# nsdumont/Semantic-Spiking-Neural-SLAM-2023

Measured on AMD Instinct MI355X. Metric: sim-sec/wall-sec, SSP-SLAM ssp_dim=1015 10k PI neurons, 1/2/4/8 MI355X, higher is better.
Workload: dtype f32; 1 GPU; PathIntegration 2-D ssp_dim=1015 pi_n_neurons=10000/VCO (508 VCOs, 5080000 LIF neurons), configs[1]; eval_points_per_vco=4000, parallelism=1 GPU, build_cache=miss

## Files before the change

semantic-spiking-neural-slam-2023_amd/csrc/ssn_block.hpp:

```cpp
#pragma once
#include <type_traits>
#include "ssn_launch.hpp"

namespace ssn {

__device__ inline float wave_sum_dpp(float v) {
  int x;
#define SSN_DPP_ADD(ctrl, rmask)                                                                             \
  x = __builtin_amdgcn_update_dpp(0, __builtin_bit_cast(int, v), ctrl, rmask, 0xF, false);                    \
  v += __builtin_bit_cast(float, x);
  SSN_DPP_ADD(0xB1, 0xF)
  SSN_DPP_ADD(0x4E, 0xF)
  SSN_DPP_ADD(0x141, 0xF)
  SSN_DPP_ADD(0x140, 0xF)
  SSN_DPP_ADD(0x142, 0xA)
  SSN_DPP_ADD(0x143, 0xC)
#undef SSN_DPP_ADD
  return v;
}
__device__ inline float row_sum_dpp(float v) {
  int x;
#define SSN_DPP_ADD(ctrl)                                                                                    \
  x = __builtin_amdgcn_update_dpp(0, __builtin_bit_cast(int, v), ctrl, 0xF, 0xF, false);                      \
  v += __builtin_bit_cast(float, x);
// ... 10 lines not shown
  }
  SSN_DPP_STAGE(0xB1, 0xF) SSN_DPP_STAGE(0x4E, 0xF) SSN_DPP_STAGE(0x141, 0xF) SSN_DPP_STAGE(0x140, 0xF)
  SSN_DPP_STAGE(0x142, 0xA) SSN_DPP_STAGE(0x143, 0xC)
#undef SSN_DPP_STAGE
}
__device__ inline double wave_sum_dpp(double v) {
#pragma unroll
  for (int off = 32; off > 0; off >>= 1) v += __shfl_xor(v, off, 64);
  return v;
}
template <int N>
__device__ inline void wave_sum_dpp_n(double* v) {
#pragma unroll
  for (int r = 0; r < N; ++r) v[r] = wave_sum_dpp(v[r]);
}

typedef float f32x2 __attribute__((ext_vector_type(2)));
typedef unsigned int u32x2 __attribute__((ext_vector_type(2)));
__device__ inline f32x2 pk_clamp01(f32x2 x) {
  f32x2 r;
  asm("v_pk_mul_f32 %0, %1, 1.0 op_sel_hi:[1,0] clamp" : "=v"(r) : "v"(x));
  return r;
}
__device__ inline f32x2 pk_sub_clamp01(f32x2 x, f32x2 y) {
  f32x2 r;
  asm("v_pk_add_f32 %0, %1, %2 neg_lo:[0,1] neg_hi:[0,1] clamp" : "=v"(r) : "v"(x), "s"(y));
  return r;
}
__device__ inline f32x2 pk_mul_clamp01(f32x2 x, f32x2 y) {
  f32x2 r;
  asm("v_pk_mul_f32 %0, %1, %2 clamp" : "=v"(r) : "v"(x), "s"(y));
  return r;
}
__device__ inline f32x2 pk_fma_clamp01_vsv(f32x2 x, f32x2 y, f32x2 z) {
  f32x2 r;
  asm("v_pk_fma_f32 %0, %1, %2, %3 clamp" : "=v"(r) : "v"(x), "s"(y), "v"(z));
  return r;
}
__device__ inline f32x2 pk_fma_clamp01_trans_vvs(f32x2 x, f32x2 y, f32x2 z) {
  f32x2 r;
  asm("s_nop 0\n\tv_pk_fma_f32 %0, %1, %2, %3 clamp" : "=v"(r) : "v"(x), "v"(y), "s"(z));
  return r;
}

__device__ inline f32x2 pk_fma_clamp01_vs_negv(f32x2 x, f32x2 y, f32x2 z) {
  f32x2 r;
  asm("v_pk_fma_f32 %0, %1, %2, %3 neg_lo:[0,0,1] neg_hi:[0,0,1] clamp" : "=v"(r) : "v"(x), "s"(y), "v"(z));
  return r;
}

struct LifConstV3 { float na, ca, m1, c1, c2, c3, p0, p1, p2, ktau_ref, K; };
struct LifConstV3P { f32x2 na, ca, m1, c1, c2, c3, p0, p1, p2, ktau_ref; };

__device__ inline LifConstV3 lif_const_v3(double dt, double tau_rc, double tau_ref) {
  double K = 1.0;
  while (2.0 * K * tau_ref <= 1.0 && K < 1048576.0) K *= 2.0;
  while (K * tau_ref > 1.0) K *= 0.5;
  const double h = dt / tau_rc;
  const double x0 = h, x1 = 0.5 * h, x2 = 0.0669872981077807 * h;
  auto f = [](double x) { return -expm1(-x) / x; };
  const double f0 = f(x0), f1 = f(x1), f2 = f(x2);
  const double d01 = (f1 - f0) / (x1 - x0), d12 = (f2 - f1) / (x2 - x1), d012 = (d12 - d01) / (x2 - x0);
  const double q2 = d012, q1 = d01 - d012 * (x0 + x1), q0 = f0 - d01 * x0 + d012 * x0 * x1;
  LifConstV3 c;
  const float a = (float)(1.0 / (K * dt));
  float ca = a + 1.0f;
  if ((double)ca < (double)a + 1.0) ca = __builtin_bit_cast(float, __builtin_bit_cast(unsigned int, ca) + 1u);
  c.na = -a; c.ca = ca; c.m1 = (float)(1.0 + K * dt);
  c.c1 = (float)(q0 * h); c.c2 = (float)(q1 * h * h); c.c3 = (float)(q2 * h * h * h);
  {
    const double um = -expm1(-h);
    const double u0 = um * 0.9330127018922193, u1 = um * 0.5, u2 = um * 0.0669872981077807;
    auto phi = [](double u) { return log1p(-u) / u; };
    const double g0 = phi(u0), g1 = phi(u1), g2 = phi(u2);
    const double e01 = (g1 - g0) / (u1 - u0), e12 = (g2 - g1) / (u2 - u1), e012 = (e12 - e01) / (u2 - u0);
    const double r2 = e012, r1 = e01 - e012 * (u0 + u1), r0 = g0 - e01 * u0 + e012 * u0 * u1;
    c.p0 = (float)(K * tau_rc * r0); c.p1 = (float)(K * tau_rc * r1); c.p2 = (float)(K * tau_rc * r2);
  }
  c.ktau_ref = (float)(K * tau_ref); c.K = (float)K;
  return c;
}

__device__ inline f32x2 lif_state_dl(f32x2 w, f32x2 na, f32x2 ca) {
  return pk_fma_clamp01_vsv(w, (f32x2)(na), (f32x2)(ca));
}
__device__ inline f32x2 lif_state_p1(f32x2 dl, f32x2 c3, f32x2 c2) {
  f32x2 P;
  asm("v_pk_fma_f32 %0, %1, %2, %3" : "=v"(P) : "v"(dl), "v"((f32x2)(c3)), "s"((f32x2)(c2)));
  return P;
}
__device__ inline f32x2 lif_state_p2(f32x2 dl, f32x2 P, f32x2 c1) {
  asm("v_pk_fma_f32 %0, %1, %2, %3" : "=v"(P) : "v"(dl), "v"(P), "s"((f32x2)(c1)));
  return P;
}
__device__ inline void lif_state_part(f32x2 w, const LifConstV3P& c, f32x2& W0, f32x2& em) {
  W0 = pk_clamp01(w);
  const f32x2 dl = lif_state_dl(w, c.na, c.ca);
  const f32x2 P = lif_state_p2(dl, lif_state_p1(dl, c.c3, c.c2), c.c1);
  em = dl * P;
}
__device__ inline f32x2 lif_spike_test(f32x2 Jm1, f32x2 w, f32x2 W0, f32x2 em, const LifConstV3P& c, f32x2 big, f32x2& U, f32x2& nmt) {
  nmt = pk_sub_clamp01(w, (f32x2)(c.m1));
  U = __builtin_elementwise_fma(Jm1 + W0, em, -W0);
  return pk_mul_clamp01(U, big);
}
__device__ inline void lif_finish_spiking(f32x2 Jm1, f32x2& w, f32x2 U, f32x2 nmt, f32x2 spk, const LifConstV3P& c, f32x2 big) {
  f32x2 rc;
  rc.x = __builtin_amdgcn_rcpf(Jm1.x);
  rc.y = __builtin_amdgcn_rcpf(Jm1.y);
  const f32x2 u = U * rc;
  f32x2 P, nu;
  asm("v_pk_fma_f32 %0, %1, %2, %3" : "=v"(P) : "v"(u), "v"((f32x2)(c.p2)), "s"((f32x2)(c.p1)));
  asm("v_pk_fma_f32 %0, %1, %2, %3" : "=v"(P) : "v"(u), "v"(P), "s"((f32x2)(c.p0)));
  asm("v_pk_fma_f32 %0, %1, %2, %3 clamp" : "=v"(nu) : "v"(u), "v"(P), "s"((f32x2)(c.ktau_ref)));
  const f32x2 Wn = pk_fma_clamp01_vs_negv(spk, big, U);
  w = __builtin_elementwise_fma(spk, nu, Wn + nmt);
}
__device__ inline void lif_finish_silent(f32x2& w, f32x2 U, f32x2 nmt) {
  f32x2 Wn;
  asm("v_pk_mul_f32 %0, %1, -1.0 op_sel_hi:[1,0] clamp" : "=v"(Wn) : "v"(U));
  w = Wn + nmt;
}
__device__ inline f32x2 lif_input_part(f32x2 Jm1, f32x2& w, f32x2 W0, f32x2 em, const LifConstV3P& c, f32x2 big) {
  const f32x2 nmt = pk_sub_clamp01(w, (f32x2)(c.m1));
  const f32x2 U = __builtin_elementwise_fma(Jm1 + W0, em, -W0);
  const f32x2 spk = pk_mul_clamp01(U, big);
  f32x2 rc;
  rc.x = __builtin_amdgcn_rcpf(Jm1.x);
  rc.y = __builtin_amdgcn_rcpf(Jm1.y);
  f32x2 Wn, u, P, nu;
  asm("v_pk_fma_f32 %0, %2, %3, %4 neg_lo:[0,0,1] neg_hi:[0,0,1] clamp\n\t"
      "v_pk_mul_f32 %1, %4, %5"
      : "=&v"(Wn), "=v"(u)
      : "v"(spk), "s"(big), "v"(U), "v"(rc));
  asm("v_pk_fma_f32 %0, %1, %2, %3" : "=v"(P) : "v"(u), "v"((f32x2)(c.p2)), "s"((f32x2)(c.p1)));
  asm("v_pk_fma_f32 %0, %1, %2, %3" : "=v"(P) : "v"(u), "v"(P), "s"((f32x2)(c.p0)));
  asm("v_pk_fma_f32 %0, %1, %2, %3 clamp" : "=v"(nu) : "v"(u), "v"(P), "s"((f32x2)(c.ktau_ref)));
  w = __builtin_elementwise_fma(spk, nu, Wn + nmt);
  return spk;
}
__device__ inline float lif_word_in(float s, float K) { return __builtin_fmaf(-s, s < 0.0f ? K : 1.0f, 1.0f); }
__device__ inline float lif_word_out(float w, float K) { return (1.0f - w) * (w > 1.0f ? 1.0f / K : 1.0f); }

__device__ inline float bits_f(unsigned int x) { return __builtin_bit_cast(float, x); }
__device__ inline unsigned int f_bits(float x) { return __builtin_bit_cast(unsigned int, x); }

#ifdef SSN_BLOCK_STAMPS
__device__ unsigned long long g_block_stamps[9];
inline hipError_t read_block_stamps(unsigned long long* out, int reset) {
  hipError_t e = hipMemcpyFromSymbol(out, HIP_SYMBOL(g_block_stamps), sizeof(unsigned long long) * 9);
  if (e == hipSuccess && reset) {
    const unsigned long long z[9] = {0, 0, 0, 0, 0, 0, 0, 0, 0};
    e = hipMemcpyToSymbol(HIP_SYMBOL(g_block_stamps), z, sizeof z);
  }
  return e;
}
#define SSN_BSTAMP(var)                                                                          \
  do {                                                                                           \
    __builtin_amdgcn_sched_barrier(0);                                                           \
    asm volatile("s_memtime %0\n\ts_waitcnt lgkmcnt(0)" : "=s"(var) :: "memory");                \
    __builtin_amdgcn_sched_barrier(0);                                                           \
  } while (0)
#define SSN_BSTAMP_ADD(i, a, b) bst[i] += (b) - (a)
#else
#define SSN_BSTAMP(var) do {} while (0)
#define SSN_BSTAMP_ADD(i, a, b) do {} while (0)
#endif

#ifndef SSN_BLOCK_SKIP
#define SSN_BLOCK_SKIP 0
#endif
#ifndef SSN_BLOCK_PIPE
#define SSN_BLOCK_PIPE 1
#endif
#ifndef SSN_BLOCK_HOIST_A
#define SSN_BLOCK_HOIST_A 2
#endif
#ifndef SSN_BLOCK_HOIST_B
#define SSN_BLOCK_HOIST_B 4
#endif
#ifndef SSN_BLOCK_HOIST_C
#define SSN_BLOCK_HOIST_C 2
#endif
struct BlockHoist { int a, b, c; };
constexpr BlockHoist block_hoist(bool pipe, int tpb, int ng) {
  if (!pipe || SSN_BLOCK_SKIP != 0) return {0, 0, 0};
  const int room = tpb <= 512 && ng >= 10 ? ng : 0;
  const int c = SSN_BLOCK_HOIST_C >= 2 && room >= 2 ? 2 : 0;
  int b = SSN_BLOCK_HOIST_B < room - c ? SSN_BLOCK_HOIST_B : room - c;
  int a_ = SSN_BLOCK_HOIST_A < room - c - b ? SSN_BLOCK_HOIST_A : room - c - b;
  return {a_, b, c};
}

template <typename T, int DIN, int DOUT, int NPT, int TPB, int LDSW, int SPLIT = 0, int TAP = 0>
__global__ __launch_bounds__(TPB) void k_ens_block(BlockArgs<T> a) {
  static_assert(!(SPLIT && TAP), "the split kernel has no tapped form");
  constexpr bool ENC_LDS = LDSW == DIN;
  static_assert(LDSW == 0 || LDSW == DIN, "LDSW");
  extern __shared__ __align__(16) unsigned char ssn_block_dyn[];
  T* const e_lds = reinterpret_cast<T*>(ssn_block_dyn);
  constexpr bool F32 = sizeof(T) == 4;
  constexpr int PK = F32 ? 2 : 1;
  constexpr int NG = NPT / PK;
  static_assert(NPT % PK == 0, "f32 variants handle neuron pairs");
  constexpr bool PIPE = F32 && NG >= 5 && SSN_BLOCK_PIPE != 0;
  constexpr BlockHoist HO = block_hoist(PIPE, TPB, NG);
  constexpr int HC = HO.c, HA = HO.a, HB = HO.b, HT = HC + HA + HB;
  using G = typename std::conditional<F32, f32x2, T>::type;
  constexpr int DP = DOUT <= 4 ? 4 : 8;
  static_assert(!SPLIT || (sizeof(T) == 4 && DOUT <= 4), "split ensembles: f32, at most four decoded rows");
  const int P = SPLIT ? a.P : 1;
  const int k = P > 1 ? (int)blockIdx.x / P : (int)blockIdx.x;
  const int member = P > 1 ? (int)blockIdx.x - k * P : 0;
  const int noff = member * a.n_member;
  const int n_loc = P > 1 ? max(0, min(a.n_member, a.n_pad - noff)) : a.n_pad;
  const int tid = threadIdx.x;
  const int nthr = NG == 1 ? (int)blockDim.x : TPB;
  const int lane = tid & 63, wave = tid >> 6;
  const size_t row = (size_t)a.n_pad;
  const T* __restrict__ enc = a.enc + (size_t)k * DIN * row + noff;
  const T* __restrict__ bias = a.bias + (size_t)k * row + noff;
  T* __restrict__ Sp = a.S + (size_t)k * row + noff;
  const NeuronParams<T> np = a.np;
  const LifMath<T> lm(np);
  const int* tcol = nullptr;
  if constexpr (TAP != 0) {
    const int tslot = a.tap_slot[k];
    if (tslot >= 0) tcol = a.tap_col + (size_t)tslot * row;
  }
  auto uni = [](float v) { return bits_f(__builtin_amdgcn_readfirstlane(f_bits(v))); };
  const LifConstV3 lc0 = lif_const_v3((double)np.dt, (double)np.tau_rc, (double)np.tau_ref);
  auto uni2 = [&](float v) { const float u = uni(v); return (f32x2){u, u}; };
  const LifConstV3P lc = {uni2(lc0.na), uni2(lc0.ca), uni2(lc0.m1), uni2(lc0.c1), uni2(lc0.c2), uni2(lc0.c3), uni2(lc0.p0), uni2(lc0.p1),
                          uni2(lc0.p2), uni2(lc0.ktau_ref)};
  const float lcK = uni(lc0.K);
  const f32x2 big = {0x1p100f, 0x1p100f};

  G e[ENC_LDS ? 1 : NG][DIN], b[NG], s[NG], dc[NG][DOUT];
  constexpr int cap = (NG == 1 ? 1024 : TPB) * NPT;
  int lrow[LDSW > 0 ? LDSW : 1];
#pragma unroll
  for (int d = 0; d < (LDSW > 0 ? LDSW : 1); ++d) {
    lrow[d] = d * cap + tid * PK;
    asm volatile("" : "+v"(lrow[d]));
  }
  auto lds_group = [&](int d, int g) -> const G* {
    return reinterpret_cast<const G*>(e_lds + lrow[d] + g * nthr * PK);
  };
#pragma unroll
  for (int g = 0; g < NG; ++g) {
    const int i0 = (g * nthr + tid) * PK;
    const bool in = i0 < n_loc;
    const int ii = in ? i0 : 0;
    const T msk = in ? T(1) : T(0);
    auto ld = [&](const T* p) -> G { if constexpr (F32) return *reinterpret_cast<const f32x2*>(p) * msk; else return *p * msk; };
#pragma unroll
    for (int d = 0; d < DIN; ++d) {
      const G ev = ld(enc + d * row + ii);
      if constexpr (ENC_LDS) *reinterpret_cast<G*>(e_lds + d * cap + i0) = ev; else e[g][d] = ev;
    }
    b[g] = ld(bias + ii);
    s[g] = ld(Sp + ii);
    if constexpr (F32) {
      b[g] = b[g] - 1.0f;
      s[g] = (f32x2){lif_word_in(s[g].x, lcK), lif_word_in(s[g].y, lcK)};
    }
    if (a.dec_neuron_major) {
      const T* dp = a.dec + ((size_t)k * row + noff + ii) * DP;
#pragma unroll
      for (int r = 0; r < DOUT; ++r) {
        if constexpr (F32) dc[g][r] = (f32x2){dp[r], dp[DP + r]} * msk; else dc[g][r] = dp[r] * msk;
      }
    } else {
      const T* dp = a.dec + (size_t)k * DOUT * row + noff + ii;
#pragma unroll
      for (int r = 0; r < DOUT; ++r) dc[g][r] = ld(dp + r * row);
    }
  }

  constexpr int CH = 32;
  constexpr int XP = 4;
  constexpr int RW = DOUT <= 4 ? 64 : 128;
  __shared__ __align__(16) T red[2][RW];
  __shared__ __align__(16) T xs[CH][XP];
  __shared__ T os[CH][DOUT];
  __shared__ int s_dst[DOUT];
  __shared__ int s_out[DOUT];
  for (int i = tid; i < 2 * RW; i += nthr) (&red[0][0])[i] = T(0);
// ... 50 lines not shown
      for (int d = 0; d < LDSW; ++d) en[u][d] = *lds_group(d, u);
  }
#ifdef SSN_BLOCK_STAMPS
  unsigned long long bst[6] = {0, 0, 0, 0, 0, 0}, bt0 = 0, bt1 = 0, bt2 = 0, bt3 = 0, bt4 = 0, bt5 = 0, bt6 = 0, bm0 = 0, br0 = 0;
  asm volatile("s_memtime %0\n\ts_memrealtime %1\n\ts_waitcnt lgkmcnt(0)" : "=s"(bm0), "=s"(br0) :: "memory");
#endif
  unsigned int n_slots = 0, n_silent = 0;
  T x[DIN];
  int xl[DIN];
#pragma unroll
  for (int d = 0; d < DIN; ++d) xl[d] = __builtin_amdgcn_readfirstlane((xr[d] & 3) << 4);
  auto assemble_x = [&](const float4 xv) {
    const float xin[4] = {xv.x, xv.y, xv.z, xv.w};
    float f1 = 0.0f;
    if constexpr (DOUT > 4) f1 = bits_f(__builtin_amdgcn_readlane(f_bits(F1), 0));
#pragma unroll
    for (int d = 0; d < DIN; ++d) {
      const float f0 = bits_f(__builtin_amdgcn_readlane(f_bits(F0), xl[d]));
      float st = f0;
      if constexpr (DOUT > 4) st = xr[d] >= 4 ? f1 : f0;
      x[d] = __builtin_fmaf(xa[d], st, xin[d]);
    }
  };
  f32x2 W0h[HT > 0 ? HT : 1], emh[HT > 0 ? HT : 1];
  if constexpr (HT > 0) {
#pragma unroll
    for (int g = 0; g < HT; ++g) lif_state_part(s[g], lc, W0h[g], emh[g]);
  }
  for (int j0 = 0; j0 < a.B; j0 += CH) {
    const int cn = min(CH, a.B - j0);
    __syncthreads();
    if (j0 > 0 && member == 0) {
      for (int i = tid; i < CH * DOUT; i += nthr) {
        const int jj = i / DOUT, r = i - jj * DOUT;
        if (s_out[r]) a.bsig[(size_t)(a.row0 + j0 - CH + jj) * a.n_sig + s_dst[r]] = os[jj][r];
      }
    }
    for (int i = tid; i < cn * DIN; i += nthr) {
      const int jj = i / DIN, d = i - jj * DIN;
      xs[jj][d] = xbase[(size_t)(j0 + jj) * a.n_sig + d];
    }
    __syncthreads();
    if constexpr (PIPE) {
      assemble_x(*(const float4*)xs[0]);
    }

    for (int jj = 0; jj < cn; ++jj) {
      SSN_BSTAMP(bt0);
      if constexpr (SPLIT != 0) {
        if (P > 1 && wave == 0 && (lane & 15) == 0) {
// ... 32 lines not shown
          for (int d = 0; d < DIN; ++d) {
            if constexpr (ENC_LDS) J[u] += en[u][d] * x[d];
            else J[u] += e[g][d] * x[d];
          }
        }
        if constexpr (ENC_LDS) {
#pragma unroll
          for (int u = 0; u < IL; ++u) {
            if (g0 + u >= NG) continue;
            asm volatile("" : "+v"(J[u]));
            const int gn = g0 + IL + u < NG ? g0 + IL + u : (g0 + IL + u) % IL;
#pragma unroll
            for (int d = 0; d < LDSW; ++d) en[u][d] = *lds_group(d, gn);
          }
        }
        bool at_rest = false;
        if constexpr (F32 && SSN_BLOCK_SKIP == 2) {
          ++n_slots;
          f32x2 r2 = {0.0f, 0.0f};
#pragma unroll
          for (int u = 0; u < IL; ++u) {
            if (g0 + u >= NG) continue;
            f32x2 pj;
            asm("v_pk_add_f32 %0, %1, 1.0 op_sel_hi:[1,0] clamp" : "=v"(pj) : "v"(J[u]));
            const f32x2 q = s[g0 + u] - 1.0f;
            r2 += __builtin_elementwise_fma(q, q, pj);
          }
          at_rest = __builtin_amdgcn_ballot_w64(__builtin_bit_cast(unsigned long long, r2) != 0ull) == 0ull;
          if (at_rest) ++n_silent;
        }
        if constexpr (F32 && SSN_BLOCK_SKIP == 1) {
          ++n_slots;
          f32x2 Uu[IL], nm[IL];
          f32x2 any2 = {0.0f, 0.0f};
#pragma unroll
          for (int u = 0; u < IL; ++u) {
            const int g = g0 + u < NG ? g0 + u : NG - 1;
            f32x2 W0, em;
            lif_state_part(s[g], lc, W0, em);
            spk[u] = lif_spike_test(J[u], s[g], W0, em, lc, big, Uu[u], nm[u]);
            if (g0 + u < NG) any2 += spk[u];
          }
          if (__builtin_amdgcn_ballot_w64(any2.x + any2.y != 0.0f) != 0ull) {
#pragma unroll
            for (int u = 0; u < IL; ++u)
              if (g0 + u < NG) lif_finish_spiking(J[u], s[g0 + u], Uu[u], nm[u], spk[u], lc, big);
#pragma unroll
            for (int u = 0; u < IL; ++u) {
              if (g0 + u >= NG) continue;
#pragma unroll
              for (int r = 0; r < DOUT; ++r) accg[r] = __builtin_elementwise_fma(spk[u], dc[g0 + u][r], accg[r]);
            }
          } else {
#pragma unroll
            for (int u = 0; u < IL; ++u)
              if (g0 + u < NG) lif_finish_silent(s[g0 + u], Uu[u], nm[u]);
            ++n_silent;
          }
        }
        if (!at_rest) {
#pragma unroll
        for (int u = 0; u < IL; ++u) {
          const int g = g0 + u;
          if (g >= NG) continue;
          if constexpr (F32 && SSN_BLOCK_SKIP == 1) {
          } else if constexpr (F32) {
            f32x2 W0, em;
            if (g < HT) { W0 = W0h[g < HT ? g : 0]; em = emh[g < HT ? g : 0]; }
            else lif_state_part(s[g], lc, W0, em);
            spk[u] = lif_input_part(J[u], s[g], W0, em, lc, big);
          } else {
            const T sw = s[g];
            T V = sw < T(0) ? T(0) : sw;
            T R = (sw < T(0) ? -sw : T(0)) - np.dt;
            T delta = np.dt - R;
            delta = delta < T(0) ? T(0) : (delta > np.dt ? np.dt : delta);
            V = V - (J[u] - V) * lm.decay(delta);
            spk[u] = T(0);
            if (V > T(1)) {
              const T t_spike = np.dt + np.tau_rc * lm.spike_time_term(V, J[u]);
              R = np.tau_ref + t_spike;
              V = T(0);
              spk[u] = T(1);
            } else if (V < T(0)) {
              V = T(0);
            }
            s[g] = R > np.dt ? -R : V;
          }
        }
#pragma unroll
        for (int u = 0; u < IL; ++u) {
          const int g = g0 + u;
          if (g >= NG) continue;
// ... 40 lines not shown
          const auto p01 = __builtin_amdgcn_permlane32_swap(f_bits(acc[0]), f_bits(acc[1]), false, false);
          const auto p23 = __builtin_amdgcn_permlane32_swap(f_bits(acc[2]), f_bits(acc[3]), false, false);
          const float s01 = bits_f(p01[0]) + bits_f(p01[1]);
          const float s23 = bits_f(p23[0]) + bits_f(p23[1]);
          const auto q = __builtin_amdgcn_permlane16_swap(f_bits(s01), f_bits(s23), false, false);
          float t4 = bits_f(q[0]) + bits_f(q[1]);
          t4 = row_sum_dpp(t4);
          if constexpr (DOUT == 5) {
            const float w4 = wave_sum_dpp(acc[4]);
            if (wslot >= 0) red[par][wslot] = lane == 63 ? w4 : t4;
          } else {
            if (wslot >= 0) red[par][wslot] = t4;
          }
        } else {
          wave_sum_dpp_n<DOUT>(acc);
          if (lane == 63) {
#pragma unroll
            for (int r = 0; r < DOUT; ++r) red[par][r * 16 + wave] = acc[r];
          }
        }
        if constexpr (HA > 0) {
          __builtin_amdgcn_sched_barrier(0);
#pragma unroll
          for (int g = HC; g < HC + HA; ++g) lif_state_part(s[g], lc, W0h[g], emh[g]);
          __builtin_amdgcn_sched_barrier(0);
        }
        SSN_BSTAMP(bt3);
        __syncthreads();
        SSN_BSTAMP(bt4);
        if constexpr (PIPE) {
          const float rv = red[par][lane];
          float rv1 = 0.0f;
          if constexpr (DOUT > 4) rv1 = red[par][64 + lane];
          if constexpr (HB > 0) {
            __builtin_amdgcn_sched_barrier(0);
#pragma unroll
            for (int g = HC + HA; g < HT; ++g) lif_state_part(s[g], lc, W0h[g], emh[g]);
            __builtin_amdgcn_sched_barrier(0);
          }
          if constexpr (HC == 2) {
            f32x2 dl0, dl1, P0, P1;
            v0 = rv;
            asm volatile(
                "v_pk_fma_f32 %1, %7, %9, %10 clamp\n\t"
                "v_pk_fma_f32 %2, %8, %9, %10 clamp\n\t"
                "v_add_f32_dpp %0, %0, %0 quad_perm:[1,0,3,2] row_mask:0xf bank_mask:0xf bound_ctrl:1\n\t"
                "v_pk_fma_f32 %3, %1, %11, %12\n\t"
                "v_pk_fma_f32 %4, %2, %11, %12\n\t"
                "v_add_f32_dpp %0, %0, %0 quad_perm:[2,3,0,1] row_mask:0xf bank_mask:0xf bound_ctrl:1\n\t"
                "v_pk_fma_f32 %3, %1, %3, %13\n\t"
                "v_pk_fma_f32 %4, %2, %4, %13\n\t"
                "v_add_f32_dpp %0, %0, %0 row_half_mirror row_mask:0xf bank_mask:0xf bound_ctrl:1\n\t"
                "v_pk_mul_f32 %5, %1, %3\n\t"
                "v_pk_mul_f32 %6, %2, %4\n\t"
                "v_add_f32_dpp %0, %0, %0 row_mirror row_mask:0xf bank_mask:0xf bound_ctrl:1"
                : "+v"(v0), "=&v"(dl0), "=&v"(dl1), "=&v"(P0), "=&v"(P1), "=&v"(emh[0]), "=&v"(emh[1])
                : "v"(s[0]), "v"(s[1]), "s"(lc.na), "v"(lc.ca), "v"(lc.c3), "s"(lc.c2), "s"(lc.c1));
          } else {
            v0 = row_sum_dpp(rv);
          }
          if constexpr (DOUT > 4) v1 = rv1;
        } else {
          v0 = row_sum_dpp(red[par][lane]);
        }
        SSN_BSTAMP(bt5);
        if constexpr (SPLIT != 0) {
          if (P > 1) {
            const int tq = j0 + jj;
            unsigned int* const xb = a.xslots + (size_t)k * 64;
            const size_t bstride = (size_t)a.K * 64;
            if (wave == 0 && (lane & 15) == 0) {
              unsigned int* const pub = xb + (size_t)(tq % 3) * bstride + member * 4 + (lane >> 4);
              const unsigned int val = f_bits(v0);
              asm volatile("s_waitcnt vmcnt(0)\n\tglobal_store_dword %0, %1, off sc0 sc1" :: "v"(pub), "v"(val) : "memory");
            }
            const unsigned int* const src = xb + (size_t)(tq % 3) * bstride + (lane & 15) * 4 + (lane >> 4);
            const bool mine = (lane & 15) < P;
            unsigned int got = 0, spins = 0;
            while (true) {
              if (mine) asm volatile("global_load_dword %0, %1, off sc0 sc1\n\ts_waitcnt vmcnt(0)" : "=v"(got) : "v"(src) : "memory");
              if (!__any(mine && got == BLOCK_XCHG_SENTINEL)) break;
              if (++spins > (1u << 20)) { if (lane == 0) *a.xerr = 1; break; }
            }
            v0 = row_sum_dpp(mine ? bits_f(got) : 0.0f);
          }
        }
        F0 = __builtin_fmaf(la0, F0, lb0 * v0);
        if constexpr (HC > 0) {
          __builtin_amdgcn_sched_barrier(0);
#pragma unroll
          for (int g = 0; g < HC; ++g) W0h[g] = pk_clamp01(s[g]);
          __builtin_amdgcn_sched_barrier(0);
        }
        if constexpr (DOUT > 4) {
          if constexpr (PIPE) v1 = row_sum_dpp(v1); else v1 = row_sum_dpp(red[par][64 + lane]);
          F1 = __builtin_fmaf(la1, F1, lb1 * v1);
        }
        if constexpr (PIPE) assemble_x(xnx);
        if (wave == 0 && member == 0) {
          if ((lane & 15) == 0 && (lane >> 4) < DOUT) os[jj][lane >> 4] = v0;
          if (DOUT > 4 && lane == 0) os[jj][4] = v1;
        }
        SSN_BSTAMP(bt6);
        SSN_BSTAMP_ADD(0, bt0, bt1); SSN_BSTAMP_ADD(1, bt1, bt2); SSN_BSTAMP_ADD(2, bt2, bt3); SSN_BSTAMP_ADD(3, bt3, bt4);
        SSN_BSTAMP_ADD(4, bt4, bt6); SSN_BSTAMP_ADD(5, bt4, bt5);
      } else {
        T acc[DOUT];
#pragma unroll
        for (int r = 0; r < DOUT; ++r) acc[r] = accg[r];
        wave_sum_dpp_n<DOUT>(acc);
        if (lane == 63) {
#pragma unroll
          for (int r = 0; r < DOUT; ++r) red[par][r * 16 + wave] = acc[r];
        }
// ... 28 lines not shown
    }
  }
#endif
  if constexpr (F32 && SSN_BLOCK_SKIP != 0) {
    if (lane == 0 && a.slot_stats) {
      atomicAdd(a.slot_stats, (unsigned long long)n_slots);
      atomicAdd(a.slot_stats + 1, (unsigned long long)n_silent);
    }
  }
  __syncthreads();
  if (member == 0) {
    const int j0 = (a.B - 1) / CH * CH, cn = a.B - j0;
    for (int i = tid; i < cn * DOUT; i += nthr) {
      const int jj = i / DOUT, r = i - jj * DOUT;
      if (s_out[r]) a.bsig[(size_t)(a.row0 + j0 + jj) * a.n_sig + s_dst[r]] = os[jj][r];
    }
  }

  int tid2 = tid;
  asm volatile("" : "+v"(tid2));
#pragma unroll
  for (int g = 0; g < NG; ++g) {
    const int i0 = (g * nthr + tid2) * PK;
    if constexpr (F32) s[g] = (f32x2){lif_word_out(s[g].x, lcK), lif_word_out(s[g].y, lcK)};
    if (i0 < n_loc) *reinterpret_cast<G*>(Sp + i0) = s[g];
  }
  if constexpr (TAP != 0) {
    if (tcol && a.B > 0) {
      const T* const lrow = a.bsig + (size_t)(a.row0 + a.B - 1) * a.n_sig;
#pragma unroll
      for (int g = 0; g < NG; ++g) {
        const int i0 = (g * nthr + tid2) * PK;
        if (i0 >= n_loc) continue;
#pragma unroll
        for (int c = 0; c < PK; ++c) {
          const int d = tcol[i0 + c];
          if (d >= 0) a.sig_w[d] = lrow[d];
        }
      }
    }
  }
  if (a.B > 0 && member == 0) {
    if constexpr (F32) {
      if (wave == 0 && (lane & 15) == 0 && (lane >> 4) < DOUT) {
        const int r = lane >> 4;
        a.sig_w[s_dst[r]] = v0;
        const int st = a.lp_state[(long long)k * DOUT + r];
// ... 101 lines not shown
```

semantic-spiking-neural-slam-2023_amd/csrc/ssn_host.hip:

```cpp
#include <hip/hip_runtime.h>
#include <dlfcn.h>
#include <algorithm>
#include <climits>
#include <cmath>
#include <cstdarg>
#include <cstdio>
#include <cstdlib>
#include <cstring>
#include <memory>
#include <mutex>
#include <map>
#include <set>
#include <string>
#include <thread>
#include <vector>

#include "../../include/ssn.h"
#include "ssn_launch.hpp"
#include "ssn_recall.hpp"

namespace {

__global__ void k_set_block(ssn::StepCtx* ctx, long long block_start) { ctx->block_start = block_start; }
__global__ void k_advance(ssn::StepCtx* ctx, long long n) { ctx->step += n; }
// ... 1272 lines not shown
      CHK(dupload(&t.ro, rowout));
      CHK(upload(lp_a.data(), t.a, 1, nr, nr));
      CHK(upload(lp_b.data(), t.b, 1, nr, nr));
      if (!with_x) return SSN_OK;
      CHK(dupload(&t.xrow, xrow));
      CHK(dmalloc(&t.xalpha, K * din * (int64_t)sizeof(T)));
      CHK(upload(xalpha.data(), t.xalpha, 1, K * din, K * din));
      return SSN_OK;
    };
    int blk_threads = 0, blk_tpb = 0, blk_npt = 0, blk_lds = 0;
    int split_P = 1, n_member = 0;
    if (opt.has(SSN_PLAN_SPLIT_BLOCK) && sizeof(T) == 4 && dout <= 4) {
      hipDeviceProp_t prop;
      int n_cu = 256;
      if (hipGetDeviceProperties(&prop, device) == hipSuccess) n_cu = prop.multiProcessorCount;
      if (opt.block_split_cus != PlanOptions::UNSET) n_cu = opt.block_split_cus;
      const int64_t n_ens = eo.i[2];
      for (int cand : {4, 2}) {
        if (K * cand <= n_cu && n_ens / cand >= 1024) { split_P = cand; break; }
      }
      { const int q = opt.block_split; if (q == 1 || q == 2 || q == 4 || q == 8) split_P = q; }
      if (split_P > 1) n_member = (int)(((n_ens + split_P - 1) / split_P + 3) / 4 * 4);
    }
    if (defer && !drv && !opt.has(SSN_PLAN_NO_BLOCK_KERNEL) && ens_fast(eo) && (sizeof(T) == 8 || (dt <= 0.05 * eo.f[0] && eo.f[1] >= dt)) &&
        ssn::ens_block_supported<T>((int)din, (int)dout, split_P > 1 ? n_member : (int)eo.i[2], opt.block_variant.v, &blk_threads, &blk_tpb, &blk_npt, &blk_lds)) {
      FilterTabs ft;
      CHK(filter_tables(ft, true));
      ssn::EnsArgs<T> ea;
      fill_ens_args(eo, taps, drv, ea);
      blk = ssn::BlockArgs<T>{};
      blk.enc = ea.enc; blk.bias = ea.bias; blk.dec = ea.dec; blk.S = ea.V;
      blk.xrows = bsig; blk.bsig = bsig; blk.sig = sig; blk.sig_w = sig;
      blk.didx = (const int*)bufs[eo.i[8]].d; blk.lp_state = ft.lp; blk.lp_a = ft.a; blk.lp_b = ft.b;
      blk.xrow = ft.xrow; blk.xalpha = ft.xalpha; blk.rowout = ft.ro;
      blk.n_sig = n_sig; blk.x_off = eo.i[0];
      blk.K = ea.K; blk.n = ea.n; blk.n_pad = ea.n_pad; blk.din = ea.din; blk.dout = ea.dout;
      blk.B = 0; blk.row0 = 1; blk.threads = blk_threads; blk.tpb = blk_tpb; blk.npt = blk_npt; blk.enc_lds = blk_lds;
      blk.dec_neuron_major = ea.fast == 1 ? 1 : 0;
      blk.np = ea.np;
      blk.P = split_P; blk.n_member = n_member; blk.xslots = nullptr; blk.xerr = nullptr;
      {
        unsigned long long* d_ss = nullptr;
        CHK(dzeros(&d_ss, 2));
        blk.slot_stats = d_ss;
      }
      if (split_P > 1) {
        unsigned int* d_x = nullptr; int* d_e = nullptr;
// ... 2414 lines not shown
```

semantic-spiking-neural-slam-2023_amd/csrc/ssn_launch.hpp:

```cpp
#pragma once
#include <hip/hip_runtime.h>
#include <stdint.h>
#include <atomic>

namespace ssn {

inline hipError_t set_max_dynamic_lds_once(const void* fn, int bytes, std::atomic<uint64_t>& done) {
  int dev = 0;
  hipError_t e = hipGetDevice(&dev);
  if (e != hipSuccess) return e;
  const uint64_t bit = 1ull << (dev & 63);
  if (done.load(std::memory_order_acquire) & bit) return hipSuccess;
  e = hipFuncSetAttribute(fn, hipFuncAttributeMaxDynamicSharedMemorySize, bytes);
  if (e == hipSuccess) done.fetch_or(bit, std::memory_order_release);
  return e;
}

template <typename T>
struct NeuronParams {
  int type;
  T dt, tau_rc, tau_ref, min_voltage;
};

struct StepCtx;
// ... 221 lines not shown
  const MicroOp<T>* mops;
  const int* chain;
  const unsigned char* arena;
  T* sig;
  StepCtx* ctx;
  RoundEntry e[MAX_ROUND_ENTRIES];
};
template <typename T> hipError_t launch_round(hipStream_t, const RoundArgs<T>&, int n_blocks, size_t lds_bytes);
constexpr int GLUE_CHUNK = 1024;
constexpr int GLUE_ROWS = 256;

constexpr int MAX_BATCH_OPS = 24;
template <typename T> struct BatchOpList { BatchOp<T> op[MAX_BATCH_OPS]; int count; };
template <typename T> hipError_t launch_batch_elementwise(hipStream_t, const BatchOpList<T>&);

template <typename T> hipError_t launch_ensarray(hipStream_t, const EnsArgs<T>&);
template <typename T> hipError_t launch_ensarray_batch(hipStream_t, const EnsBatch<T>&, int count);
template <typename T> hipError_t launch_dec_pack(hipStream_t, const T* src, T* dst, int K, int dout, int n, int n_pad, int DP, int unpack);
template <typename T> hipError_t launch_state_unpack(hipStream_t, const T* src, T* out, int64_t n, int want_refractory, T r_offset);
template <typename T> hipError_t launch_ens_finish(hipStream_t, const FinishArgs<T>&);
template <typename T> hipError_t launch_dft(hipStream_t, const DftBatch&, int count);
template <typename T> hipError_t launch_ens_block(hipStream_t, const BlockArgs<T>&);
template <typename T> bool ens_block_supported(int din, int dout, int n, const int want[3], int* threads, int* tpb, int* npt, int* enc_lds);
template <typename T> hipError_t launch_program(hipStream_t, const MicroOp<T>* ops, const ProgDesc* progs, int n_progs, T* sig, StepCtx* ctx);
template <typename T> hipError_t launch_vecops(hipStream_t, const MicroOp<T>* ops, int n_ops, int wgs, T* sig, const StepCtx* ctx);
template <typename T> hipError_t launch_matvec(hipStream_t, const MatvecBatch<T>&, int count);
template <typename T> hipError_t launch_matvec_ordered(hipStream_t, const T* Wt, const T* x, T* y, int rows, int cols, int ldt);
template <typename T> hipError_t launch_transpose(hipStream_t, const T* src, T* dst, int rows, int cols, int ld, int ldt);
template <typename T> hipError_t launch_spmv_partial(hipStream_t, const SpmvBatch<T>&, int count);
template <typename T> hipError_t launch_neurons(hipStream_t, const NeuronsBatch<T>&, int count);
template <typename T> hipError_t launch_pes(hipStream_t, T* W, const T* err, const T* act, int rows, int cols, int ld, T kappa);
template <typename T> hipError_t launch_voja(hipStream_t, T* E, const T* spk, const T* key, const T* learn, const T* scale,
                                            int rows, int cols, int ld, T lr_dt);
template <typename T> hipError_t launch_batch_op(hipStream_t, const BatchOp<T>&);
template <typename T> hipError_t launch_argmax_partial(hipStream_t, const T* sims, long long n, T* out, int P, int nsplit);
template <typename T> hipError_t launch_grid_lhs(hipStream_t, const T* X, const T* E, int lde, T* A, int lda, int na, int K);
template <typename T> hipError_t launch_gemm_nt(hipStream_t, const T* A, int lda, const T* Wm, int ldw, T* C, int ldc, int M, int N, int K, int splits);
template <typename T> hipError_t launch_convert_in(hipStream_t, const double* src, T* dst, int64_t rows, int64_t cols, int64_t ld);
template <typename T> hipError_t launch_convert_out(hipStream_t, const T* src, double* dst, int64_t rows, int64_t cols, int64_t ld);

}
```

Before: 361.5 sim-sec/wall-sec.

## Reformulate LIF state update as affine exponential-domain map to drop polynomial evaluations

Replaces the LIF neuron state encoding with an exponentially transformed (affine) representation. The per-step membrane and refractory updates then become fused multiply-adds instead of quadratic polynomial approximations of expm1 and log1p. Encoders and bias are prescaled by E1 at load, and the conversion cost moves to the kernel entry and exit via expf and log1pf on the stored state. The hoisting scheme is reworked to precompute dl and nmt rather than the em product, and the hand-written DPP-interleaved asm block is dropped. A host-side guard keeps the block kernel only when the kappa scaling gives enough precision, which risks falling back to the slower path for some parameter sets.

```diff
diff --git a/semantic-spiking-neural-slam-2023_amd/csrc/ssn_block.hpp b/semantic-spiking-neural-slam-2023_amd/csrc/ssn_block.hpp
--- a/semantic-spiking-neural-slam-2023_amd/csrc/ssn_block.hpp
+++ b/semantic-spiking-neural-slam-2023_amd/csrc/ssn_block.hpp
@@ -56,11 +56,6 @@
   asm("v_pk_mul_f32 %0, %1, 1.0 op_sel_hi:[1,0] clamp" : "=v"(r) : "v"(x));
   return r;
 }
-__device__ inline f32x2 pk_sub_clamp01(f32x2 x, f32x2 y) {
-  f32x2 r;
-  asm("v_pk_add_f32 %0, %1, %2 neg_lo:[0,1] neg_hi:[0,1] clamp" : "=v"(r) : "v"(x), "s"(y));
-  return r;
-}
 __device__ inline f32x2 pk_mul_clamp01(f32x2 x, f32x2 y) {
   f32x2 r;
   asm("v_pk_mul_f32 %0, %1, %2 clamp" : "=v"(r) : "v"(x), "s"(y));
@@ -77,77 +72,48 @@
   return r;
 }
 
-__device__ inline f32x2 pk_fma_clamp01_vs_negv(f32x2 x, f32x2 y, f32x2 z) {
-  f32x2 r;
-  asm("v_pk_fma_f32 %0, %1, %2, %3 neg_lo:[0,0,1] neg_hi:[0,0,1] clamp" : "=v"(r) : "v"(x), "s"(y), "v"(z));
-  return r;
-}
-
-struct LifConstV3 { float na, ca, m1, c1, c2, c3, p0, p1, p2, ktau_ref, K; };
-struct LifConstV3P { f32x2 na, ca, m1, c1, c2, c3, p0, p1, p2, ktau_ref; };
-
-__device__ inline LifConstV3 lif_const_v3(double dt, double tau_rc, double tau_ref) {
-  double K = 1.0;
-  while (2.0 * K * tau_ref <= 1.0 && K < 1048576.0) K *= 2.0;
-  while (K * tau_ref > 1.0) K *= 0.5;
-  const double h = dt / tau_rc;
-  const double x0 = h, x1 = 0.5 * h, x2 = 0.0669872981077807 * h;
-  auto f = [](double x) { return -expm1(-x) / x; };
-  const double f0 = f(x0), f1 = f(x1), f2 = f(x2);
-  const double d01 = (f1 - f0) / (x1 - x0), d12 = (f2 - f1) / (x2 - x1), d012 = (d12 - d01) / (x2 - x0);
-  const double q2 = d012, q1 = d01 - d012 * (x0 + x1), q0 = f0 - d01 * x0 + d012 * x0 * x1;
-  LifConstV3 c;
-  const float a = (float)(1.0 / (K * dt));
+struct LifConstA { float q, nqm1, E1, A, nB, na, c, kq, rkq, tau_rc, rtau_rc; };
+struct LifConstAP { f32x2 q, nqm1, E1, A, nB, na, c; };
+
+__device__ inline LifConstA lif_const_affine(double dt, double tau_rc, double tau_ref) {
+  const double h = dt / tau_rc, q = exp(-h), E1 = -expm1(-h), C1 = exp((tau_ref - dt) / tau_rc);
+  const double kappa = lif_affine_kappa(dt, tau_rc, tau_ref);
+  LifConstA c;
+  const float a = (float)(1.0 / (kappa * E1));
   float ca = a + 1.0f;
   if ((double)ca < (double)a + 1.0) ca = __builtin_bit_cast(float, __builtin_bit_cast(unsigned int, ca) + 1u);
-  c.na = -a; c.ca = ca; c.m1 = (float)(1.0 + K * dt);
-  c.c1 = (float)(q0 * h); c.c2 = (float)(q1 * h * h); c.c3 = (float)(q2 * h * h * h);
-  {
-    const double um = -expm1(-h);
-    const double u0 = um * 0.9330127018922193, u1 = um * 0.5, u2 = um * 0.0669872981077807;
-    auto phi = [](double u) { return log1p(-u) / u; };
-    const double g0 = phi(u0), g1 = phi(u1), g2 = phi(u2);
-    const double e01 = (g1 - g0) / (u1 - u0), e12 = (g2 - g1) / (u2 - u1), e012 = (e12 - e01) / (u2 - u0);
-    const double r2 = e012, r1 = e01 - e012 * (u0 + u1), r0 = g0 - e01 * u0 + e012 * u0 * u1;
-    c.p0 = (float)(K * tau_rc * r0); c.p1 = (float)(K * tau_rc * r1); c.p2 = (float)(K * tau_rc * r2);
-  }
-  c.ktau_ref = (float)(K * tau_ref); c.K = (float)K;
+  c.na = -a; c.c = ca;
+  c.q = (float)q; c.nqm1 = (float)(-q * (1.0 + kappa * E1)); c.E1 = (float)E1;
+  c.A = (float)(kappa * (C1 - q)); c.nB = (float)(-kappa * C1 * E1);
+  c.kq = (float)(kappa * q); c.rkq = (float)(1.0 / (kappa * q)); c.tau_rc = (float)tau_rc; c.rtau_rc = (float)(1.0 / tau_rc);
   return c;
 }
 
 __device__ inline f32x2 lif_state_dl(f32x2 w, f32x2 na, f32x2 ca) {
   return pk_fma_clamp01_vsv(w, (f32x2)(na), (f32x2)(ca));
 }
-__device__ inline f32x2 lif_state_p1(f32x2 dl, f32x2 c3, f32x2 c2) {
-  f32x2 P;
-  asm("v_pk_fma_f32 %0, %1, %2, %3" : "=v"(P) : "v"(dl), "v"((f32x2)(c3)), "s"((f32x2)(c2)));
-  return P;
-}
-__device__ inline f32x2 lif_state_p2(f32x2 dl, f32x2 P, f32x2 c1) {
-  asm("v_pk_fma_f32 %0, %1, %2, %3" : "=v"(P) : "v"(dl), "v"(P), "s"((f32x2)(c1)));
-  return P;
-}
-__device__ inline void lif_state_part(f32x2 w, const LifConstV3P& c, f32x2& W0, f32x2& em) {
+__device__ inline f32x2 lif_state_nmt(f32x2 w, f32x2 q, f32x2 nqm1) {
+  return pk_fma_clamp01_vsv(w, (f32x2)(q), (f32x2)(nqm1));
+}
+__device__ inline void lif_state_part(f32x2 w, const LifConstAP& c, f32x2& W0, f32x2& dl) {
   W0 = pk_clamp01(w);
-  const f32x2 dl = lif_state_dl(w, c.na, c.ca);
-  const f32x2 P = lif_state_p2(dl, lif_state_p1(dl, c.c3, c.c2), c.c1);
-  em = dl * P;
-}
-__device__ inline f32x2 lif_spike_test(f32x2 Jm1, f32x2 w, f32x2 W0, f32x2 em, const LifConstV3P& c, f32x2 big, f32x2& U, f32x2& nmt) {
-  nmt = pk_sub_clamp01(w, (f32x2)(c.m1));
-  U = __builtin_elementwise_fma(Jm1 + W0, em, -W0);
+  dl = lif_state_dl(w, c.na, c.c);
+}
+__device__ inline f32x2 lif_spike_test(f32x2 JE, f32x2 W0, f32x2 dl, const LifConstAP& c, f32x2 big, f32x2& U) {
+  const f32x2 t = __builtin_elementwise_fma(W0, c.E1, JE);
+  U = __builtin_elementwise_fma(t, dl, -W0);
   return pk_mul_clamp01(U, big);
 }
-__device__ inline void lif_finish_spiking(f32x2 Jm1, f32x2& w, f32x2 U, f32x2 nmt, f32x2 spk, const LifConstV3P& c, f32x2 big) {
+__device__ inline void lif_finish_spiking(f32x2 JE, f32x2& w, f32x2 U, f32x2 nmt, f32x2 spk, const LifConstAP& c, f32x2 big) {
   f32x2 rc;
-  rc.x = __builtin_amdgcn_rcpf(Jm1.x);
-  rc.y = __builtin_amdgcn_rcpf(Jm1.y);
-  const f32x2 u = U * rc;
-  f32x2 P, nu;
-  asm("v_pk_fma_f32 %0, %1, %2, %3" : "=v"(P) : "v"(u), "v"((f32x2)(c.p2)), "s"((f32x2)(c.p1)));
-  asm("v_pk_fma_f32 %0, %1, %2, %3" : "=v"(P) : "v"(u), "v"(P), "s"((f32x2)(c.p0)));
-  asm("v_pk_fma_f32 %0, %1, %2, %3 clamp" : "=v"(nu) : "v"(u), "v"(P), "s"((f32x2)(c.ktau_ref)));
-  const f32x2 Wn = pk_fma_clamp01_vs_negv(spk, big, U);
+  rc.x = __builtin_amdgcn_rcpf(JE.x);
+  rc.y = __builtin_amdgcn_rcpf(JE.y);
+  f32x2 Wn, u, nu;
+  asm("v_pk_fma_f32 %0, %2, %3, %4 neg_lo:[0,0,1] neg_hi:[0,0,1] clamp\n\t"
+      "v_pk_mul_f32 %1, %4, %5"
+      : "=&v"(Wn), "=v"(u)
+      : "v"(spk), "s"(big), "v"(U), "v"(rc));
+  asm("v_pk_fma_f32 %0, %1, %2, %3 clamp" : "=v"(nu) : "v"(u), "s"((f32x2)(c.nB)), "v"((f32x2)(c.A)));
   w = __builtin_elementwise_fma(spk, nu, Wn + nmt);
 }
 __device__ inline void lif_finish_silent(f32x2& w, f32x2 U, f32x2 nmt) {
@@ -155,26 +121,18 @@
   asm("v_pk_mul_f32 %0, %1, -1.0 op_sel_hi:[1,0] clamp" : "=v"(Wn) : "v"(U));
   w = Wn + nmt;
 }
-__device__ inline f32x2 lif_input_part(f32x2 Jm1, f32x2& w, f32x2 W0, f32x2 em, const LifConstV3P& c, f32x2 big) {
-  const f32x2 nmt = pk_sub_clamp01(w, (f32x2)(c.m1));
-  const f32x2 U = __builtin_elementwise_fma(Jm1 + W0, em, -W0);
-  const f32x2 spk = pk_mul_clamp01(U, big);
-  f32x2 rc;
-  rc.x = __builtin_amdgcn_rcpf(Jm1.x);
-  rc.y = __builtin_amdgcn_rcpf(Jm1.y);
-  f32x2 Wn, u, P, nu;
-  asm("v_pk_fma_f32 %0, %2, %3, %4 neg_lo:[0,0,1] neg_hi:[0,0,1] clamp\n\t"
-      "v_pk_mul_f32 %1, %4, %5"
-      : "=&v"(Wn), "=v"(u)
-      : "v"(spk), "s"(big), "v"(U), "v"(rc));
-  asm("v_pk_fma_f32 %0, %1, %2, %3" : "=v"(P) : "v"(u), "v"((f32x2)(c.p2)), "s"((f32x2)(c.p1)));
-  asm("v_pk_fma_f32 %0, %1, %2, %3" : "=v"(P) : "v"(u), "v"(P), "s"((f32x2)(c.p0)));
-  asm("v_pk_fma_f32 %0, %1, %2, %3 clamp" : "=v"(nu) : "v"(u), "v"(P), "s"((f32x2)(c.ktau_ref)));
-  w = __builtin_elementwise_fma(spk, nu, Wn + nmt);
+__device__ inline f32x2 lif_input_part(f32x2 JE, f32x2& w, f32x2 W0, f32x2 dl, f32x2 nmt, const LifConstAP& c, f32x2 big) {
+  f32x2 U;
+  const f32x2 spk = lif_spike_test(JE, W0, dl, c, big, U);
+  lif_finish_spiking(JE, w, U, nmt, spk, c, big);
   return spk;
 }
-__device__ inline float lif_word_in(float s, float K) { return __builtin_fmaf(-s, s < 0.0f ? K : 1.0f, 1.0f); }
-__device__ inline float lif_word_out(float w, float K) { return (1.0f - w) * (w > 1.0f ? 1.0f / K : 1.0f); }
+__device__ inline float lif_word_in(float s, float kq, float rtau_rc) {
+  return s < 0.0f ? __builtin_fmaf(kq, expm1f(-s * rtau_rc), 1.0f) : 1.0f - s;
+}
+__device__ inline float lif_word_out(float w, float rkq, float tau_rc) {
+  return w > 1.0f ? -(tau_rc * log1pf((w - 1.0f) * rkq)) : 1.0f - w;
+}
 
 __device__ inline float bits_f(unsigned int x) { return __builtin_bit_cast(float, x); }
 __device__ inline unsigned int f_bits(float x) { return __builtin_bit_cast(unsigned int, x); }
@@ -213,17 +171,20 @@
 #ifndef SSN_BLOCK_HOIST_B
 #define SSN_BLOCK_HOIST_B 4
 #endif
-#ifndef SSN_BLOCK_HOIST_C
-#define SSN_BLOCK_HOIST_C 2
-#endif
-struct BlockHoist { int a, b, c; };
+#ifndef SSN_BLOCK_HOIST_D
+#define SSN_BLOCK_HOIST_D 1
+#endif
+#ifndef SSN_BLOCK_HOIST_NMT
+#define SSN_BLOCK_HOIST_NMT 1
+#endif
+struct BlockHoist { int a, b, d; };
 constexpr BlockHoist block_hoist(bool pipe, int tpb, int ng) {
   if (!pipe || SSN_BLOCK_SKIP != 0) return {0, 0, 0};
   const int room = tpb <= 512 && ng >= 10 ? ng : 0;
-  const int c = SSN_BLOCK_HOIST_C >= 2 && room >= 2 ? 2 : 0;
-  int b = SSN_BLOCK_HOIST_B < room - c ? SSN_BLOCK_HOIST_B : room - c;
-  int a_ = SSN_BLOCK_HOIST_A < room - c - b ? SSN_BLOCK_HOIST_A : room - c - b;
-  return {a_, b, c};
+  const int d = SSN_BLOCK_HOIST_D < room ? SSN_BLOCK_HOIST_D : room;
+  const int b = SSN_BLOCK_HOIST_B < room - d ? SSN_BLOCK_HOIST_B : room - d;
+  const int a_ = SSN_BLOCK_HOIST_A < room - d - b ? SSN_BLOCK_HOIST_A : room - d - b;
+  return {a_, b, d};
 }
 
 template <typename T, int DIN, int DOUT, int NPT, int TPB, int LDSW, int SPLIT = 0, int TAP = 0>
@@ -239,7 +200,8 @@
   static_assert(NPT % PK == 0, "f32 variants handle neuron pairs");
   constexpr bool PIPE = F32 && NG >= 5 && SSN_BLOCK_PIPE != 0;
   constexpr BlockHoist HO = block_hoist(PIPE, TPB, NG);
-  constexpr int HC = HO.c, HA = HO.a, HB = HO.b, HT = HC + HA + HB;
+  constexpr int HD = HO.d, HA = HO.a, HB = HO.b, HT = HD + HA + HB;
+  constexpr bool HNMT = SSN_BLOCK_HOIST_NMT != 0;
   using G = typename std::conditional<F32, f32x2, T>::type;
   constexpr int DP = DOUT <= 4 ? 4 : 8;
   static_assert(!SPLIT || (sizeof(T) == 4 && DOUT <= 4), "split ensembles: f32, at most four decoded rows");
@@ -263,11 +225,10 @@
     if (tslot >= 0) tcol = a.tap_col + (size_t)tslot * row;
   }
   auto uni = [](float v) { return bits_f(__builtin_amdgcn_readfirstlane(f_bits(v))); };
-  const LifConstV3 lc0 = lif_const_v3((double)np.dt, (double)np.tau_rc, (double)np.tau_ref);
+  const LifConstA lc0 = lif_const_affine((double)np.dt, (double)np.tau_rc, (double)np.tau_ref);
   auto uni2 = [&](float v) { const float u = uni(v); return (f32x2){u, u}; };
-  const LifConstV3P lc = {uni2(lc0.na), uni2(lc0.ca), uni2(lc0.m1), uni2(lc0.c1), uni2(lc0.c2), uni2(lc0.c3), uni2(lc0.p0), uni2(lc0.p1),
-                          uni2(lc0.p2), uni2(lc0.ktau_ref)};
-  const float lcK = uni(lc0.K);
+  const LifConstAP lc = {uni2(lc0.q), uni2(lc0.nqm1), uni2(lc0.E1), uni2(lc0.A), uni2(lc0.nB), uni2(lc0.na), uni2(lc0.c)};
+  const float lcE1 = uni(lc0.E1), lcKq = uni(lc0.kq), lcRkq = uni(lc0.rkq), lcTau = uni(lc0.tau_rc), lcRtau = uni(lc0.rtau_rc);
   const f32x2 big = {0x1p100f, 0x1p100f};
 
   G e[ENC_LDS ? 1 : NG][DIN], b[NG], s[NG], dc[NG][DOUT];
@@ -290,14 +251,15 @@
     auto ld = [&](const T* p) -> G { if constexpr (F32) return *reinterpret_cast<const f32x2*>(p) * msk; else return *p * msk; };
 #pragma unroll
     for (int d = 0; d < DIN; ++d) {
-      const G ev = ld(enc + d * row + ii);
+      G ev = ld(enc + d * row + ii);
+      if constexpr (F32) ev = ev * lcE1;
       if constexpr (ENC_LDS) *reinterpret_cast<G*>(e_lds + d * cap + i0) = ev; else e[g][d] = ev;
     }
     b[g] = ld(bias + ii);
     s[g] = ld(Sp + ii);
     if constexpr (F32) {
-      b[g] = b[g] - 1.0f;
-      s[g] = (f32x2){lif_word_in(s[g].x, lcK), lif_word_in(s[g].y, lcK)};
+      b[g] = (b[g] - 1.0f) * lcE1;
+      s[g] = (f32x2){lif_word_in(s[g].x, lcKq, lcRtau), lif_word_in(s[g].y, lcKq, lcRtau)};
     }
     if (a.dec_neuron_major) {
       const T* dp = a.dec + ((size_t)k * row + noff + ii) * DP;
@@ -394,10 +356,14 @@
       x[d] = __builtin_fmaf(xa[d], st, xin[d]);
     }
   };
-  f32x2 W0h[HT > 0 ? HT : 1], emh[HT > 0 ? HT : 1];
+  f32x2 W0h[HT > 0 ? HT : 1], dlh[HT > 0 ? HT : 1], nmth[HT > 0 ? HT : 1];
+  auto hoist_state = [&](int g) {
+    lif_state_part(s[g], lc, W0h[g], dlh[g]);
+    if constexpr (HNMT) nmth[g] = lif_state_nmt(s[g], lc.q, lc.nqm1);
+  };
   if constexpr (HT > 0) {
 #pragma unroll
-    for (int g = 0; g < HT; ++g) lif_state_part(s[g], lc, W0h[g], emh[g]);
+    for (int g = 0; g < HT; ++g) hoist_state(g);
   }
   for (int j0 = 0; j0 < a.B; j0 += CH) {
     const int cn = min(CH, a.B - j0);
@@ -476,7 +442,7 @@
           for (int u = 0; u < IL; ++u) {
             if (g0 + u >= NG) continue;
             f32x2 pj;
-            asm("v_pk_add_f32 %0, %1, 1.0 op_sel_hi:[1,0] clamp" : "=v"(pj) : "v"(J[u]));
+            asm("v_pk_add_f32 %0, %1, %2 clamp" : "=v"(pj) : "v"(J[u]), "s"(lc.E1));
             const f32x2 q = s[g0 + u] - 1.0f;
             r2 += __builtin_elementwise_fma(q, q, pj);
           }
@@ -490,9 +456,10 @@
 #pragma unroll
           for (int u = 0; u < IL; ++u) {
             const int g = g0 + u < NG ? g0 + u : NG - 1;
-            f32x2 W0, em;
-            lif_state_part(s[g], lc, W0, em);
-            spk[u] = lif_spike_test(J[u], s[g], W0, em, lc, big, Uu[u], nm[u]);
+            f32x2 W0, dl;
+            lif_state_part(s[g], lc, W0, dl);
+            nm[u] = lif_state_nmt(s[g], lc.q, lc.nqm1);
+            spk[u] = lif_spike_test(J[u], W0, dl, lc, big, Uu[u]);
             if (g0 + u < NG) any2 += spk[u];
           }
           if (__builtin_amdgcn_ballot_w64(any2.x + any2.y != 0.0f) != 0ull) {
@@ -519,10 +486,12 @@
           if (g >= NG) continue;
           if constexpr (F32 && SSN_BLOCK_SKIP == 1) {
           } else if constexpr (F32) {
-            f32x2 W0, em;
-            if (g < HT) { W0 = W0h[g < HT ? g : 0]; em = emh[g < HT ? g : 0]; }
-            else lif_state_part(s[g], lc, W0, em);
-            spk[u] = lif_input_part(J[u], s[g], W0, em, lc, big);
+            f32x2 W0, dl, nmt;
+            if (g < HT) { W0 = W0h[g < HT ? g : 0]; dl = dlh[g < HT ? g : 0]; }
+            else lif_state_part(s[g], lc, W0, dl);
+            if (HNMT && g < HT) nmt = nmth[g < HT ? g : 0];
+            else nmt = lif_state_nmt(s[g], lc.q, lc.nqm1);
+            spk[u] = lif_input_part(J[u], s[g], W0, dl, nmt, lc, big);
           } else {
             const T sw = s[g];
             T V = sw < T(0) ? T(0) : sw;
@@ -609,7 +578,7 @@
         if constexpr (HA > 0) {
           __builtin_amdgcn_sched_barrier(0);
 #pragma unroll
-          for (int g = HC; g < HC + HA; ++g) lif_state_part(s[g], lc, W0h[g], emh[g]);
+          for (int g = HD; g < HD + HA; ++g) hoist_state(g);
           __builtin_amdgcn_sched_barrier(0);
         }
         SSN_BSTAMP(bt3);
@@ -622,30 +591,10 @@
           if constexpr (HB > 0) {
             __builtin_amdgcn_sched_barrier(0);
 #pragma unroll
-            for (int g = HC + HA; g < HT; ++g) lif_state_part(s[g], lc, W0h[g], emh[g]);
+            for (int g = HD + HA; g < HT; ++g) hoist_state(g);
             __builtin_amdgcn_sched_barrier(0);
           }
-          if constexpr (HC == 2) {
-            f32x2 dl0, dl1, P0, P1;
-            v0 = rv;
-            asm volatile(
-                "v_pk_fma_f32 %1, %7, %9, %10 clamp\n\t"
-                "v_pk_fma_f32 %2, %8, %9, %10 clamp\n\t"
-                "v_add_f32_dpp %0, %0, %0 quad_perm:[1,0,3,2] row_mask:0xf bank_mask:0xf bound_ctrl:1\n\t"
-                "v_pk_fma_f32 %3, %1, %11, %12\n\t"
-                "v_pk_fma_f32 %4, %2, %11, %12\n\t"
-                "v_add_f32_dpp %0, %0, %0 quad_perm:[2,3,0,1] row_mask:0xf bank_mask:0xf bound_ctrl:1\n\t"
-                "v_pk_fma_f32 %3, %1, %3, %13\n\t"
-                "v_pk_fma_f32 %4, %2, %4, %13\n\t"
-                "v_add_f32_dpp %0, %0, %0 row_half_mirror row_mask:0xf bank_mask:0xf bound_ctrl:1\n\t"
-                "v_pk_mul_f32 %5, %1, %3\n\t"
-                "v_pk_mul_f32 %6, %2, %4\n\t"
-                "v_add_f32_dpp %0, %0, %0 row_mirror row_mask:0xf bank_mask:0xf bound_ctrl:1"
-                : "+v"(v0), "=&v"(dl0), "=&v"(dl1), "=&v"(P0), "=&v"(P1), "=&v"(emh[0]), "=&v"(emh[1])
-                : "v"(s[0]), "v"(s[1]), "s"(lc.na), "v"(lc.ca), "v"(lc.c3), "s"(lc.c2), "s"(lc.c1));
-          } else {
-            v0 = row_sum_dpp(rv);
-          }
+          v0 = row_sum_dpp(rv);
           if constexpr (DOUT > 4) v1 = rv1;
         } else {
           v0 = row_sum_dpp(red[par][lane]);
@@ -673,10 +622,10 @@
           }
         }
         F0 = __builtin_fmaf(la0, F0, lb0 * v0);
-        if constexpr (HC > 0) {
+        if constexpr (HD > 0) {
           __builtin_amdgcn_sched_barrier(0);
 #pragma unroll
-          for (int g = 0; g < HC; ++g) W0h[g] = pk_clamp01(s[g]);
+          for (int g = 0; g < HD; ++g) hoist_state(g);
           __builtin_amdgcn_sched_barrier(0);
         }
         if constexpr (DOUT > 4) {
@@ -751,7 +700,7 @@
 #pragma unroll
   for (int g = 0; g < NG; ++g) {
     const int i0 = (g * nthr + tid2) * PK;
-    if constexpr (F32) s[g] = (f32x2){lif_word_out(s[g].x, lcK), lif_word_out(s[g].y, lcK)};
+    if constexpr (F32) s[g] = (f32x2){lif_word_out(s[g].x, lcRkq, lcTau), lif_word_out(s[g].y, lcRkq, lcTau)};
     if (i0 < n_loc) *reinterpret_cast<G*>(Sp + i0) = s[g];
   }
   if constexpr (TAP != 0) {
diff --git a/semantic-spiking-neural-slam-2023_amd/csrc/ssn_host.hip b/semantic-spiking-neural-slam-2023_amd/csrc/ssn_host.hip
--- a/semantic-spiking-neural-slam-2023_amd/csrc/ssn_host.hip
+++ b/semantic-spiking-neural-slam-2023_amd/csrc/ssn_host.hip
@@ -1318,7 +1318,7 @@
       { const int q = opt.block_split; if (q == 1 || q == 2 || q == 4 || q == 8) split_P = q; }
       if (split_P > 1) n_member = (int)(((n_ens + split_P - 1) / split_P + 3) / 4 * 4);
     }
-    if (defer && !drv && !opt.has(SSN_PLAN_NO_BLOCK_KERNEL) && ens_fast(eo) && (sizeof(T) == 8 || (dt <= 0.05 * eo.f[0] && eo.f[1] >= dt)) &&
+    if (defer && !drv && !opt.has(SSN_PLAN_NO_BLOCK_KERNEL) && ens_fast(eo) && (sizeof(T) == 8 || (dt <= 0.05 * eo.f[0] && eo.f[1] >= dt && ssn::lif_affine_kappa((double)(T)dt, (double)(T)eo.f[0], (double)(T)eo.f[1]) >= 4.0)) &&
         ssn::ens_block_supported<T>((int)din, (int)dout, split_P > 1 ? n_member : (int)eo.i[2], opt.block_variant.v, &blk_threads, &blk_tpb, &blk_npt, &blk_lds)) {
       FilterTabs ft;
       CHK(filter_tables(ft, true));
diff --git a/semantic-spiking-neural-slam-2023_amd/csrc/ssn_launch.hpp b/semantic-spiking-neural-slam-2023_amd/csrc/ssn_launch.hpp
--- a/semantic-spiking-neural-slam-2023_amd/csrc/ssn_launch.hpp
+++ b/semantic-spiking-neural-slam-2023_amd/csrc/ssn_launch.hpp
@@ -267,6 +267,12 @@
 template <typename T> hipError_t launch_dft(hipStream_t, const DftBatch&, int count);
 template <typename T> hipError_t launch_ens_block(hipStream_t, const BlockArgs<T>&);
 template <typename T> bool ens_block_supported(int din, int dout, int n, const int want[3], int* threads, int* tpb, int* npt, int* enc_lds);
+__host__ __device__ inline double lif_affine_kappa(double dt, double tau_rc, double tau_ref) {
+  const double span = exp((tau_ref - dt) / tau_rc) - exp(-dt / tau_rc);
+  double kappa = 1048576.0;
+  while (kappa * span > 1.0 && kappa > 0x1p-20) kappa *= 0.5;
+  return kappa;
+}
 template <typename T> hipError_t launch_program(hipStream_t, const MicroOp<T>* ops, const ProgDesc* progs, int n_progs, T* sig, StepCtx* ctx);
 template <typename T> hipError_t launch_vecops(hipStream_t, const MicroOp<T>* ops, int n_ops, int wgs, T* sig, const StepCtx* ctx);
 template <typename T> hipError_t launch_matvec(hipStream_t, const MatvecBatch<T>&, int count);
```

New measurement: 401.5 sim-sec/wall-sec (median of 6 runs). +11.0%, better.
